# Nicolo2277/Vivim

Measured on AMD Instinct MI355X. Metric: frames/sec fwd+bwd, 256x256 clip=5 3-class, higher is better.
Workload: dtype bf16

## Files before the change

### include/vivim_hip.h

```cpp
#ifndef VIVIM_HIP_H
#define VIVIM_HIP_H

#include <stddef.h>
#include <stdint.h>

#ifdef __cplusplus
extern "C" {
#endif

#define VIVIM_ABI_VERSION 8

typedef enum { VIVIM_F32 = 0, VIVIM_F16 = 1, VIVIM_BF16 = 2 } vivim_dtype_t;

enum {
    VIVIM_OK = 0,
    VIVIM_ERR_INVALID = 1,
    VIVIM_ERR_UNSUPPORTED = 2,
    VIVIM_ERR_LAUNCH = 3
};

typedef struct {
    int32_t batch, dim, seqlen, dstate, n_groups;
    int32_t itype;
    int32_t is_variable_B;
// ... 139 lines not shown
    const void *z;
    const void *dt_bias;
    void *out;
} vivim_state_update_params;

typedef struct {
    int32_t batch, seqlen, channels;
    int32_t itype, otype;
    float eps;
    int64_t x_batch_stride, x_c_stride;
    int64_t y_batch_stride, y_token_stride;
    int64_t dx_batch_stride, dx_c_stride;
    const void *x;
    const void *weight, *bias;
    void *y;
    void *mean, *rstd;
    const void *dy;
    void *dx;
    void *dweight, *dbias;
    void *workspace;
} vivim_layernorm_params;

typedef struct {
    int32_t groups, m, n, k;
    int32_t itype;
    int32_t _pad0;
    int64_t a_group_stride, a_row_stride;
    int64_t b_group_stride, b_row_stride;
    int64_t out_group_stride, out_row_stride;
    const void *a, *b;
    void *out;
} vivim_wgrad_nt_params;

int vivim_abi_version(void);
const char *vivim_last_error(void);

size_t vivim_sizeof(int which);

int vivim_scan_ckpt_len(const vivim_ssm_fwd_params *f);
int vivim_scan_chunk_len(int itype);

size_t vivim_scan_bwd_workspace_bytes(const vivim_ssm_fwd_params *f);
size_t vivim_scan_fwd_workspace_bytes(const vivim_ssm_fwd_params *f);

int vivim_set_tuning(int which, int value);

int vivim_selective_scan_fwd(const vivim_ssm_fwd_params *p, void *stream);
int vivim_selective_scan_bwd(const vivim_ssm_bwd_params *p, void *stream);
int vivim_causal_conv1d_fwd(const vivim_conv_fwd_params *p, void *stream);
int vivim_causal_conv1d_bwd(const vivim_conv_bwd_params *p, void *stream);
int vivim_dwconv_fwd(const vivim_dwconv_params *p, void *stream);
int vivim_dwconv_wgrad(const vivim_dwconv_wgrad_params *p, void *stream);
int vivim_dir_scatter(const vivim_dir_params *p, void *stream);
int vivim_dir_gather(const vivim_dir_params *p, void *stream);
int vivim_causal_conv1d_update(const vivim_conv_update_params *p, void *stream);
int vivim_selective_state_update(const vivim_state_update_params *p, void *stream);
int vivim_layernorm_cm_fwd(const vivim_layernorm_params *p, void *stream);
int vivim_layernorm_cm_bwd(const vivim_layernorm_params *p, void *stream);
size_t vivim_layernorm_bwd_workspace_bytes(const vivim_layernorm_params *p);
int vivim_wgrad_nt(const vivim_wgrad_nt_params *p, void *stream);

size_t vivim_scan_bwd_det_workspace_bytes(const vivim_ssm_fwd_params *f);
size_t vivim_scan_bwd_det_call_workspace_bytes(const vivim_ssm_bwd_params *p);
int vivim_selective_scan_bwd_det(const vivim_ssm_bwd_params *p, void *det_ws, size_t det_ws_bytes, void *stream);

size_t vivim_causal_conv1d_bwd_det_workspace_bytes(const vivim_conv_fwd_params *f);
int vivim_causal_conv1d_bwd_det(const vivim_conv_bwd_params *p, void *det_ws, size_t det_ws_bytes, void *stream);
size_t vivim_dwconv_wgrad_det_workspace_bytes(const vivim_dwconv_wgrad_params *p);
int vivim_dwconv_wgrad_det(const vivim_dwconv_wgrad_params *p, void *det_ws, size_t det_ws_bytes, void *stream);

#ifdef __cplusplus
}
#endif
#endif
```

### vivim_amd/_lib.py

```python
import ctypes
import os
import subprocess

_HERE = os.path.dirname(os.path.abspath(__file__))
CSRC = os.path.join(_HERE, "csrc")
SO_PATH = os.environ.get("VIVIM_LIB") or os.path.join(CSRC, "libvivim_hip.so")

i32, i64, vp = ctypes.c_int32, ctypes.c_int64, ctypes.c_void_p

F32, F16, BF16 = 0, 1, 2


class SsmFwdParams(ctypes.Structure):
    _fields_ = (
        [(n, i32) for n in ("batch", "dim", "seqlen", "dstate", "n_groups", "itype", "is_variable_B",
                            "is_variable_C", "delta_softplus", "_pad0")]
        + [(n, i64) for n in ("u_batch_stride", "u_d_stride", "delta_batch_stride", "delta_d_stride",
                              "z_batch_stride", "z_d_stride", "out_batch_stride", "out_d_stride",
                              "out_z_batch_stride", "out_z_d_stride", "A_d_stride", "A_dstate_stride",
                              "B_batch_stride", "B_group_stride", "B_dstate_stride",
                              "C_batch_stride", "C_group_stride", "C_dstate_stride")]
        + [(n, vp) for n in ("u", "delta", "A", "B", "C", "D", "delta_bias", "z", "out", "out_z", "x", "workspace")]
        + [("workspace_bytes", i64)]
    )
# ... 58 lines not shown


class ConvUpdateParams(ctypes.Structure):
    _fields_ = ([(n, i32) for n in ("batch", "dim", "width", "itype", "wtype", "silu_activation")]
                + [(n, i64) for n in ("x_batch_stride", "x_c_stride", "state_batch_stride", "state_c_stride",
                                      "state_w_stride", "weight_c_stride", "weight_width_stride",
                                      "out_batch_stride", "out_c_stride")]
                + [(n, vp) for n in ("x", "conv_state", "weight", "bias", "out")])


class StateUpdateParams(ctypes.Structure):
    _fields_ = ([(n, i32) for n in ("batch", "dim", "dstate", "itype", "stype", "dt_softplus")]
                + [(n, i64) for n in ("state_batch_stride", "state_d_stride", "state_n_stride", "x_batch_stride",
                                      "x_d_stride", "dt_batch_stride", "dt_d_stride", "A_d_stride", "A_n_stride",
                                      "B_batch_stride", "B_n_stride", "C_batch_stride", "C_n_stride",
                                      "z_batch_stride", "z_d_stride", "out_batch_stride", "out_d_stride")]
                + [(n, vp) for n in ("state", "x", "dt", "A", "B", "C", "D", "z", "dt_bias", "out")])


class LayerNormParams(ctypes.Structure):
    _fields_ = ([(n, i32) for n in ("batch", "seqlen", "channels", "itype", "otype")] + [("eps", ctypes.c_float)]
                + [(n, i64) for n in ("x_batch_stride", "x_c_stride", "y_batch_stride", "y_token_stride",
                                      "dx_batch_stride", "dx_c_stride")]
                + [(n, vp) for n in ("x", "weight", "bias", "y", "mean", "rstd", "dy", "dx", "dweight", "dbias", "workspace")])


class WgradNtParams(ctypes.Structure):
    _fields_ = ([(n, i32) for n in ("groups", "m", "n", "k", "itype", "_pad0")]
                + [(n, i64) for n in ("a_group_stride", "a_row_stride", "b_group_stride", "b_row_stride",
                                      "out_group_stride", "out_row_stride")]
                + [(n, vp) for n in ("a", "b", "out")])


EXPORTS = ("vivim_abi_version", "vivim_last_error", "vivim_scan_chunk_len", "vivim_scan_ckpt_len", "vivim_sizeof",
           "vivim_scan_bwd_workspace_bytes", "vivim_scan_fwd_workspace_bytes", "vivim_set_tuning",
           "vivim_selective_scan_fwd", "vivim_selective_scan_bwd",
           "vivim_causal_conv1d_fwd", "vivim_causal_conv1d_bwd", "vivim_dwconv_fwd", "vivim_dwconv_wgrad",
           "vivim_dir_scatter", "vivim_dir_gather", "vivim_causal_conv1d_update", "vivim_selective_state_update",
           "vivim_layernorm_cm_fwd", "vivim_layernorm_cm_bwd", "vivim_layernorm_bwd_workspace_bytes", "vivim_wgrad_nt",
           "vivim_scan_bwd_det_workspace_bytes", "vivim_scan_bwd_det_call_workspace_bytes", "vivim_selective_scan_bwd_det",
           "vivim_causal_conv1d_bwd_det_workspace_bytes", "vivim_causal_conv1d_bwd_det",
           "vivim_dwconv_wgrad_det_workspace_bytes", "vivim_dwconv_wgrad_det")

_lib = None


def build(force=False):
    if force:
        subprocess.check_call(["make", "-C", CSRC, "clean"])
    subprocess.check_call(["make", "-C", CSRC, "-j4"])
    return SO_PATH


def lib():
    global _lib
    if _lib is None:
        if not os.path.exists(SO_PATH):
            raise ImportError(
                f"{SO_PATH} is missing: run `python -c 'import __graft_entry__ as g; g.build()'` "
                "(or `make -C vivim_amd/csrc`). vivim_amd has no fallback path.")
        import torch
        L = ctypes.CDLL(SO_PATH)
        L.vivim_last_error.restype = ctypes.c_char_p
        L.vivim_sizeof.restype = ctypes.c_size_t
        L.vivim_sizeof.argtypes = [ctypes.c_int]
        L.vivim_set_tuning.restype = ctypes.c_int
        L.vivim_set_tuning.argtypes = [ctypes.c_int, ctypes.c_int]
        L.vivim_scan_ckpt_len.restype = ctypes.c_int
        L.vivim_scan_ckpt_len.argtypes = [ctypes.POINTER(SsmFwdParams)]
        for fn in (L.vivim_scan_bwd_workspace_bytes, L.vivim_scan_fwd_workspace_bytes):
            fn.restype = ctypes.c_size_t
            fn.argtypes = [ctypes.POINTER(SsmFwdParams)]
        for name, st in (("vivim_selective_scan_fwd", SsmFwdParams), ("vivim_selective_scan_bwd", SsmBwdParams),
                         ("vivim_causal_conv1d_fwd", ConvFwdParams), ("vivim_causal_conv1d_bwd", ConvBwdParams),
                         ("vivim_dwconv_fwd", DwConvParams), ("vivim_dwconv_wgrad", DwConvWgradParams),
                         ("vivim_dir_scatter", DirParams), ("vivim_dir_gather", DirParams),
                         ("vivim_causal_conv1d_update", ConvUpdateParams),
                         ("vivim_selective_state_update", StateUpdateParams),
                         ("vivim_layernorm_cm_fwd", LayerNormParams), ("vivim_layernorm_cm_bwd", LayerNormParams),
                         ("vivim_wgrad_nt", WgradNtParams)):
            fn = getattr(L, name)
            fn.argtypes = [ctypes.POINTER(st), vp]
            fn.restype = ctypes.c_int
        L.vivim_scan_bwd_det_workspace_bytes.restype = ctypes.c_size_t
        L.vivim_scan_bwd_det_workspace_bytes.argtypes = [ctypes.POINTER(SsmFwdParams)]
        for name, st in (("vivim_scan_bwd_det_call_workspace_bytes", SsmBwdParams),
                         ("vivim_causal_conv1d_bwd_det_workspace_bytes", ConvFwdParams),
                         ("vivim_dwconv_wgrad_det_workspace_bytes", DwConvWgradParams)):
            getattr(L, name).restype = ctypes.c_size_t
            getattr(L, name).argtypes = [ctypes.POINTER(st)]
        for name, st in (("vivim_selective_scan_bwd_det", SsmBwdParams), ("vivim_causal_conv1d_bwd_det", ConvBwdParams),
                         ("vivim_dwconv_wgrad_det", DwConvWgradParams)):
            getattr(L, name).argtypes = [ctypes.POINTER(st), vp, ctypes.c_size_t, vp]
            getattr(L, name).restype = ctypes.c_int
        L.vivim_layernorm_bwd_workspace_bytes.argtypes = [ctypes.POINTER(LayerNormParams)]
        L.vivim_layernorm_bwd_workspace_bytes.restype = ctypes.c_size_t
        if L.vivim_abi_version() != 8:
            raise ImportError("libvivim_hip.so ABI version mismatch")
        for which, st in enumerate((SsmFwdParams, SsmBwdParams, ConvFwdParams, ConvBwdParams, DwConvParams,
                                    DwConvWgradParams, DirParams, ConvUpdateParams, StateUpdateParams, LayerNormParams,
                                    WgradNtParams)):
            if L.vivim_sizeof(which) != ctypes.sizeof(st):
                raise ImportError(f"struct layout mismatch for {st.__name__}: "
                                  f"C {L.vivim_sizeof(which)} vs ctypes {ctypes.sizeof(st)}")
        _lib = L
    return _lib


_ISIZE = {F32: 4, F16: 2, BF16: 2}


def algorithmic_bytes(name, P):
    if name.startswith("vivim_selective_scan"):
        f = P.f if name.endswith("bwd") else P
        s = _ISIZE[f.itype]
        act = f.batch * f.dim * f.seqlen * s
        bc = (f.batch * f.n_groups * f.dstate * f.seqlen) if f.is_variable_B else f.dim * f.dstate
        has_z = bool(f.z)
        if name.endswith("fwd"):
            n_act = 3 + (2 if has_z else 0)
            return n_act * act + 2 * bc * (s if f.is_variable_B else 4) + 4 * (f.dim * f.dstate + 2 * f.dim)
        n_act = 5 + (3 if has_z else 0) + (1 if (has_z and f.out_z) else 0)
        return (n_act * act + 2 * bc * (s if f.is_variable_B else 4) + 2 * bc * 4
                + 4 * (2 * f.dim * f.dstate + 4 * f.dim))
    if name.endswith("_update"):
        return 0
    if name.startswith("vivim_dir"):
        return 4 * P.batch * P.channels * P.seqlen * _ISIZE[P.itype]
    if name.startswith("vivim_dwconv"):
        act = P.batch * P.depth * P.height * P.width * P.channels * _ISIZE[P.itype]
        return 2 * act + 4 * P.channels * (P.kd * 9 + 1)
    f = P.f if name.endswith("bwd") else P
    s = _ISIZE[f.itype]
    act = f.batch * f.dim * f.seqlen * s
    if name.endswith("fwd"):
        return 2 * act + 4 * f.dim * (f.width + 1)
    return 3 * act + 8 * f.dim * (f.width + 1)


_profile = None
_event_pool = []
_PROFILED = ("vivim_selective_scan_fwd", "vivim_selective_scan_bwd", "vivim_causal_conv1d_fwd",
             "vivim_causal_conv1d_bwd")


def profile_begin(all_kernels=False):
    global _profile
    _profile = ([], bool(all_kernels))


def profile_end():
    global _profile
    rec = _profile[0] if _profile else []
    _profile = None
    out = []
    for name, nbytes, e0, e1 in rec:
        e1.synchronize()
        out.append((name, nbytes, e0.elapsed_time(e1) * 1e-3))
        _event_pool.extend((e0, e1))
    return out

# ... 88 lines not shown
```

### vivim_amd/csrc/capi.hip

```cpp
#include <hip/hip_runtime.h>
#include <stdarg.h>
#include <stdio.h>
#include "../../include/vivim_hip.h"
#include "det.cuh"

namespace vivim {
bool conv_fwd_dispatch(const vivim_conv_fwd_params&, hipStream_t);
bool conv_bwd_dispatch(const vivim_conv_bwd_params&, hipStream_t);
bool conv_cl_fwd_dispatch(const vivim_conv_fwd_params&, hipStream_t);
bool conv_cl_bwd_dispatch(const vivim_conv_bwd_params&, hipStream_t);
bool ssm_fwd_dispatch(const vivim_ssm_fwd_params&, hipStream_t);
bool dwconv_fwd_dispatch(const vivim_dwconv_params&, hipStream_t);
bool dwconv_wgrad_dispatch(const vivim_dwconv_wgrad_params&, hipStream_t);
template <bool GATHER> bool dir_dispatch(const vivim_dir_params&, hipStream_t);
void conv_update_launch(const vivim_conv_update_params&, hipStream_t);
void state_update_launch(const vivim_state_update_params&, hipStream_t);
bool ssm_bwd_dispatch(const vivim_ssm_bwd_params&, hipStream_t);
int scan_chunk_len(int itype);
int scan_ckpt_len(const vivim_ssm_fwd_params&);
size_t scan_bwd_workspace_bytes(const vivim_ssm_fwd_params&);
size_t scan_bwd_det_workspace_bytes(const vivim_ssm_fwd_params&);
size_t scan_bwd_det_call_workspace_bytes(const vivim_ssm_bwd_params&);
size_t conv_bwd_det_slots(const vivim_conv_fwd_params&);
bool conv_bwd_det_launch(const vivim_conv_bwd_params&, hipStream_t);
size_t conv_cl_bwd_det_slots(const vivim_conv_fwd_params&);
bool conv_cl_bwd_det_launch(const vivim_conv_bwd_params&, hipStream_t);
size_t dwconv_wgrad_det_workspace_bytes(const vivim_dwconv_wgrad_params&);
int dwconv_wgrad_det_dispatch(const vivim_dwconv_wgrad_params&, void*, size_t, hipStream_t);
int ssm_bwd_det_dispatch(const vivim_ssm_bwd_params&, void* det_ws, size_t det_ws_bytes, hipStream_t);
bool layernorm_dispatch(const vivim_layernorm_params&, bool bwd, hipStream_t);
size_t layernorm_bwd_workspace_bytes(const vivim_layernorm_params&);
bool wgrad_nt_dispatch(const vivim_wgrad_nt_params&, hipStream_t);
size_t scan_fwd_workspace_bytes(const vivim_ssm_fwd_params&);
}

static thread_local char g_err[512] = "";

static int fail(int code, const char* fmt, ...) {
    va_list ap;
    va_start(ap, fmt);
    vsnprintf(g_err, sizeof(g_err), fmt, ap);
    va_end(ap);
    return code;
}

#define VCHECK(cond)                                                                   \
    do {                                                                               \
        if (!(cond)) return fail(VIVIM_ERR_INVALID, "%s: check failed: %s", __func__, #cond); \
    } while (0)

static int after_launch(const char* what) {
    const hipError_t e = hipGetLastError();
    if (e != hipSuccess) return fail(VIVIM_ERR_LAUNCH, "%s: launch failed: %s", what, hipGetErrorString(e));
    return VIVIM_OK;
}

static bool dtype_ok(int t) { return t == VIVIM_F32 || t == VIVIM_F16 || t == VIVIM_BF16; }

static int check_ssm_fwd(const vivim_ssm_fwd_params* p, bool is_bwd) {
    VCHECK(p != nullptr);
    VCHECK(dtype_ok(p->itype));
    VCHECK(p->batch > 0 && p->dim > 0 && p->seqlen > 0 && p->dstate > 0 && p->n_groups > 0);
    VCHECK(p->dstate <= 256);
    VCHECK(p->dim % p->n_groups == 0);
    VCHECK(p->u && p->delta && p->A && p->B && p->C);
// ... 27 lines not shown
}

extern "C" {

int vivim_set_tuning(int which, int value) {
    if (which < 0 || which > 1 || value < 0) return -1;
    const int prev = which == 0 ? vivim::tuning_fwd_variant() : vivim::tuning_bwd_variant();
    __atomic_store_n(&vivim::g_tune[which], value, __ATOMIC_RELAXED);
    return prev;
}
int vivim_abi_version(void) { return VIVIM_ABI_VERSION; }
const char* vivim_last_error(void) { return g_err; }
int vivim_scan_chunk_len(int itype) { return vivim::scan_chunk_len(itype); }
int vivim_scan_ckpt_len(const vivim_ssm_fwd_params* f) { return f ? vivim::scan_ckpt_len(*f) : 0; }
size_t vivim_scan_bwd_workspace_bytes(const vivim_ssm_fwd_params* f) {
    return f ? vivim::scan_bwd_workspace_bytes(*f) : 0;
}
size_t vivim_scan_fwd_workspace_bytes(const vivim_ssm_fwd_params* f) {
    return f ? vivim::scan_fwd_workspace_bytes(*f) : 0;
}
size_t vivim_sizeof(int which) {
    switch (which) {
        case 0: return sizeof(vivim_ssm_fwd_params);
        case 1: return sizeof(vivim_ssm_bwd_params);
        case 2: return sizeof(vivim_conv_fwd_params);
        case 3: return sizeof(vivim_conv_bwd_params);
        case 4: return sizeof(vivim_dwconv_params);
        case 5: return sizeof(vivim_dwconv_wgrad_params);
        case 6: return sizeof(vivim_dir_params);
        case 7: return sizeof(vivim_conv_update_params);
        case 8: return sizeof(vivim_state_update_params);
        case 9: return sizeof(vivim_layernorm_params);
        case 10: return sizeof(vivim_wgrad_nt_params);
    }
    return 0;
}

int vivim_selective_scan_fwd(const vivim_ssm_fwd_params* p, void* stream) {
    if (int rc = check_ssm_fwd(p, false)) return rc;
    if (!vivim::ssm_fwd_dispatch(*p, static_cast<hipStream_t>(stream)))
        return fail(VIVIM_ERR_UNSUPPORTED, "selective_scan_fwd not implemented for input type %d", p->itype);
    return after_launch("selective_scan_fwd");
}

static int check_ssm_bwd(const vivim_ssm_bwd_params* p) {
    VCHECK(p != nullptr);
    if (int rc = check_ssm_fwd(&p->f, true)) return rc;
    VCHECK(p->dout && p->du && p->ddelta && p->dA && p->dB && p->dC);
    VCHECK((p->f.D == nullptr) == (p->dD == nullptr));
    VCHECK((p->f.delta_bias == nullptr) == (p->ddelta_bias == nullptr));
    VCHECK((p->f.z == nullptr) == (p->dz == nullptr));
    return VIVIM_OK;
}

int vivim_selective_scan_bwd(const vivim_ssm_bwd_params* p, void* stream) {
    if (int rc = check_ssm_bwd(p)) return rc;
    if (!vivim::ssm_bwd_dispatch(*p, static_cast<hipStream_t>(stream)))
        return fail(VIVIM_ERR_UNSUPPORTED, "selective_scan_bwd not implemented for input type %d", p->f.itype);
    return after_launch("selective_scan_bwd");
}

size_t vivim_scan_bwd_det_workspace_bytes(const vivim_ssm_fwd_params* f) {
    return f && f->batch > 0 && f->dim > 0 && f->seqlen > 0 && f->dstate > 0 && f->n_groups > 0
               ? vivim::scan_bwd_det_workspace_bytes(*f) : 0;
}

// ... 226 lines not shown
}

size_t vivim_layernorm_bwd_workspace_bytes(const vivim_layernorm_params* p) {
    return p && p->batch > 0 && p->seqlen > 0 && p->channels > 0 ? vivim::layernorm_bwd_workspace_bytes(*p) : 0;
}

int vivim_layernorm_cm_bwd(const vivim_layernorm_params* p, void* stream) {
    if (int rc = check_layernorm(p)) return rc;
    VCHECK(p->dy && p->dx && (reinterpret_cast<uintptr_t>(p->dx) & 15) == 0);
    const int64_t e = p->itype == VIVIM_F32 ? 4 : 8;
    VCHECK(p->dx_batch_stride % e == 0 && p->dx_c_stride % e == 0);
    if ((p->dweight || p->dbias) && !p->workspace)
        return fail(VIVIM_ERR_INVALID, "layernorm_cm_bwd: dweight / dbias need the workspace (vivim_layernorm_bwd_workspace_bytes)");
    if (!vivim::layernorm_dispatch(*p, true, static_cast<hipStream_t>(stream)))
        return fail(VIVIM_ERR_UNSUPPORTED, "layernorm_cm_bwd not implemented for input type %d / output type %d", p->itype, p->otype);
    return after_launch("layernorm_cm_bwd");
}

int vivim_wgrad_nt(const vivim_wgrad_nt_params* p, void* stream) {
    VCHECK(p != nullptr);
    VCHECK(p->groups > 0 && p->groups <= 65535 && p->m > 0 && p->n > 0 && p->k > 0);
    VCHECK(p->a && p->b && p->out);
    if (p->itype != VIVIM_F16 && p->itype != VIVIM_BF16)
        return fail(VIVIM_ERR_UNSUPPORTED, "wgrad_nt takes f16 or bf16 operands (type %d given): f32 products stay on the library GEMM", p->itype);
    VCHECK(p->k % 8 == 0 && p->a_row_stride % 8 == 0 && p->b_row_stride % 8 == 0 && p->a_group_stride % 8 == 0 &&
           p->b_group_stride % 8 == 0);
    VCHECK((reinterpret_cast<uintptr_t>(p->a) & 15) == 0 && (reinterpret_cast<uintptr_t>(p->b) & 15) == 0);
    VCHECK((int64_t)((p->m + 63) / 64) * ((p->n + 15) / 16) <= 65535);
    if (!vivim::wgrad_nt_dispatch(*p, static_cast<hipStream_t>(stream)))
        return fail(VIVIM_ERR_UNSUPPORTED, "wgrad_nt not implemented for type %d", p->itype);
    return after_launch("wgrad_nt");
}

}
```

### vivim_amd/mamba_simple.py

```python
import math

import torch
import torch.nn as nn
import torch.nn.functional as F

import os

from .dirmap import combine_directions, stack_directions
from .causal_conv1d_interface import causal_conv1d_update
from .selective_scan_interface import mamba_inner_fn_no_out_proj, mamba_inner_grouped_fn_no_out_proj
from .selective_state_update import selective_state_update

_DIRECTIONS = ("", "_b", "_s")
_FUSED = ("conv1d{}.weight", "conv1d{}.bias", "x_proj{}.weight", "dt_proj{}.weight", "dt_proj{}.bias", "A{}_log", "D{}")


class _FusedViews(torch.autograd.Function):

    @staticmethod
    def forward(ctx, nb, *args):
        ctx.nb = nb
        return tuple(b.view_as(b) for b in args[:nb])

    @staticmethod
    def backward(ctx, *gs):
        out = [None] * (1 + ctx.nb)
        for g in gs:
            out += [None, None, None] if g is None else [g[0], g[1], g[2]]
        return tuple(out)


class Mamba(nn.Module):
    def __init__(self, d_model, d_state=16, d_conv=4, expand=2, dt_rank="auto", dt_min=0.001, dt_max=0.1,
                 dt_init="random", dt_scale=1.0, dt_init_floor=1e-4, conv_bias=True, bias=False,
                 use_fast_path=True, layer_idx=None, device=None, dtype=None, bimamba_type="none",
                 nframes=5):
        kw = {"device": device, "dtype": dtype}
        super().__init__()
        assert bimamba_type == "v3", "this fork only builds the tri-directional v3 block (mamba_simple.py:125)"
        self.d_model, self.d_state, self.d_conv, self.expand = d_model, d_state, d_conv, expand
# ... 84 lines not shown
        bufs = self._fused
        views = iter(_FusedViews.apply(len(self._fused_live), *self._fused_args))
        return [None if b is None else next(views) for b in bufs]

    def _inner(self, xz, sfx):
        conv, x_proj, dt_proj = (getattr(self, n + sfx) for n in ("conv1d", "x_proj", "dt_proj"))
        A = -torch.exp(getattr(self, f"A{sfx}_log").float())
        return mamba_inner_fn_no_out_proj(
            xz, conv.weight, conv.bias, x_proj.weight, dt_proj.weight, A, None, None,
            getattr(self, "D" + sfx).float(), delta_bias=dt_proj.bias.float(), delta_softplus=True)

    def forward(self, hidden_states, inference_params=None, nframes=None):
        if inference_params is not None:
            raise NotImplementedError("decode-time inference cache is outside Vivim's path")
        batch, seqlen, _ = hidden_states.shape
        nf = self.nframes if nframes is None else nframes
        if seqlen % nf != 0:
            raise ValueError(f"seqlen {seqlen} is not a multiple of nframes {nf}")
        xz = (self.in_proj.weight @ hidden_states.reshape(batch * seqlen, -1).t()
              ).view(2 * self.d_inner, batch, seqlen).transpose(0, 1)
        if self.in_proj.bias is not None:
            xz = xz + self.in_proj.bias.to(xz.dtype)[:, None]
        hw = seqlen // nf
        if os.environ.get("VIVIM_SEPARATE_DIRECTIONS", "0") == "1" or seqlen % 8 != 0:
            return self._forward_separate(xz, batch, seqlen, nf, hw)
        D = self.d_inner
        xz3 = stack_directions(xz, nf)
        conv_w, conv_b, x_proj_w, dt_proj_w, dt_bias, A_log, Dp = self._fused_params()
        A = -torch.exp(A_log.float()).view(3 * D, self.d_state)
        o3 = mamba_inner_grouped_fn_no_out_proj(
            xz3, conv_w.view(3 * D, self.d_conv), conv_b.view(3 * D) if conv_b is not None else None, x_proj_w, dt_proj_w,
            A, Dp.float().view(3 * D), dt_bias.float().view(3 * D), True).view(batch, 3, D, seqlen)
        y = combine_directions(o3, nf).transpose(1, 2)
        return F.linear(y, self.out_proj.weight, self.out_proj.bias)

    def _forward_separate(self, xz, batch, seqlen, nf, hw):
        out = self._inner(xz, "")
        out_b = self._inner(xz.flip([-1]), "_b").flip([-1])
        xz_s = xz.reshape(batch, 2 * self.d_inner, nf, hw).transpose(2, 3).reshape(batch, 2 * self.d_inner, seqlen)
        out_s = self._inner(xz_s, "_s")
        out_s = out_s.reshape(batch, self.d_inner, hw, nf).transpose(2, 3).reshape(batch, self.d_inner, seqlen)
        y = (out + out_b + out_s).transpose(1, 2) / 3
        return F.linear(y, self.out_proj.weight, self.out_proj.bias)

    def step(self, hidden_states, conv_state, ssm_state):
        assert hidden_states.shape[1] == 1, "Only support decoding with 1 token at a time for now"
        xz = self.in_proj(hidden_states.squeeze(1))
        x, z = xz.chunk(2, dim=-1)
        x = causal_conv1d_update(x.contiguous(), conv_state, self.conv1d.weight.squeeze(1), self.conv1d.bias, self.activation)
        x_db = self.x_proj(x)
        dt, B, C = torch.split(x_db, [self.dt_rank, self.d_state, self.d_state], dim=-1)
        dt = F.linear(dt, self.dt_proj.weight)
        A = -torch.exp(self.A_log.float())
        y = selective_state_update(ssm_state, x, dt, A, B, C, self.D, z=z, dt_bias=self.dt_proj.bias, dt_softplus=True)
        return self.out_proj(y).unsqueeze(1), conv_state, ssm_state

    def allocate_inference_cache(self, batch_size, max_seqlen, dtype=None, **kwargs):
        device = self.out_proj.weight.device
        conv_state = torch.zeros(batch_size, self.d_inner, self.d_conv, device=device,
                                 dtype=self.conv1d.weight.dtype if dtype is None else dtype)
        ssm_state = torch.zeros(batch_size, self.d_inner, self.d_state, device=device,
                                dtype=self.dt_proj.weight.dtype if dtype is None else dtype)
        return conv_state, ssm_state
```

### vivim_amd/vivim.py

```python
import math

import os

import torch
import torch.nn as nn
import torch.nn.functional as F

from . import dwconv as _dw
from . import layernorm as _ln
from .mamba_simple import Mamba


class DropPath(nn.Module):

    def __init__(self, drop_prob=0.0):
        super().__init__()
        self.drop_prob = drop_prob

    def forward(self, x):
        if self.drop_prob == 0.0 or not self.training:
            return x
        keep = 1.0 - self.drop_prob
        mask = x.new_empty((x.shape[0],) + (1,) * (x.dim() - 1)).bernoulli_(keep).div_(keep)
        return x * mask


def _init_weights(m):
    if isinstance(m, nn.Linear):
        nn.init.trunc_normal_(m.weight, std=0.02)
        if m.bias is not None:
            nn.init.constant_(m.bias, 0)
    elif isinstance(m, nn.LayerNorm):
        nn.init.constant_(m.bias, 0)
        nn.init.constant_(m.weight, 1.0)
    elif isinstance(m, nn.Conv2d):
        fan_out = m.kernel_size[0] * m.kernel_size[1] * m.out_channels // m.groups
        m.weight.data.normal_(0, math.sqrt(2.0 / fan_out))
        if m.bias is not None:
            m.bias.data.zero_()


class LayerNorm(nn.Module):
# ... 14 lines not shown
        mean = x.mean(1, keepdim=True)
        var = (x - mean).pow(2).mean(1, keepdim=True)
        x = (x - mean) / torch.sqrt(var + self.eps)
        return self.weight[:, None, None] * x + self.bias[:, None, None]


class DWConv(nn.Module):

    def __init__(self, dim=768):
        super().__init__()
        self.dwconv = nn.Conv3d(dim, dim, 3, 1, 1, bias=True, groups=dim)

    def forward(self, x, nf, H, W):
        B, _, C = x.shape
        if _dw.supported(x, self.dwconv.weight):
            return _dw.depthwise_conv_tokens(x, self.dwconv.weight, self.dwconv.bias, nf, H, W)
        x = self.dwconv(x.transpose(1, 2).view(B, C, nf, H, W))
        return x.flatten(2).transpose(1, 2)


class Mlp(nn.Module):
    def __init__(self, in_features, hidden_features=None, out_features=None, act_layer=nn.GELU, drop=0.0):
        super().__init__()
        out_features = out_features or in_features
        hidden_features = hidden_features or in_features
        self.fc1 = nn.Linear(in_features, hidden_features)
        self.dwconv = DWConv(hidden_features)
        self.act = act_layer()
        self.fc2 = nn.Linear(hidden_features, out_features)
        self.drop = nn.Dropout(drop)
        self.apply(_init_weights)

    def forward(self, x, nf, H, W):
        x = self.fc1(x)
        conv = self.dwconv.dwconv
        if isinstance(self.act, nn.GELU) and self.act.approximate == "none" and _dw.supported(x, conv.weight) \
                and not os.environ.get("VIVIM_NO_DWCONV_GELU"):
            x = self.drop(_dw.depthwise_conv_gelu_tokens(x, conv.weight, conv.bias, nf, H, W))
        else:
            x = self.drop(self.act(self.dwconv(x, nf, H, W)))
        return self.drop(self.fc2(x))


class MambaLayer(nn.Module):

    def __init__(self, dim, d_state=16, d_conv=4, expand=2, mlp_ratio=4, drop=0.0, drop_path=0.0,
                 act_layer=nn.GELU):
        super().__init__()
        self.dim = dim
        self.norm1 = nn.LayerNorm(dim)
        self.mamba = Mamba(d_model=dim, d_state=d_state, d_conv=d_conv, expand=expand, bimamba_type="v3")
        self.drop_path = DropPath(drop_path) if drop_path > 0.0 else nn.Identity()
        self.norm2 = nn.LayerNorm(dim)
        self.mlp = Mlp(in_features=dim, hidden_features=int(dim * mlp_ratio), act_layer=act_layer, drop=drop)
        self.apply(_init_weights)

    @staticmethod
    def _norm(norm, x_flat):
        if (_ln.supported(x_flat, norm.weight) and _ln.worthwhile(x_flat)
                and not os.environ.get("VIVIM_NO_FUSED_LAYERNORM")):
            return _ln.layer_norm_cm(x_flat, norm.weight, norm.bias, norm.eps)
        return norm(x_flat)

    def forward(self, x):
        B, C, nf, H, W = x.shape
        assert C == self.dim
        x_flat = x.reshape(B, C, nf * H * W).transpose(-1, -2)
        x_flat = x_flat + self.drop_path(self.mamba(self._norm(self.norm1, x_flat), nframes=nf))
        x_flat = x_flat + self.drop_path(self.mlp(self._norm(self.norm2, x_flat), nf, H, W))
        return x_flat.transpose(-1, -2).reshape(B, C, nf, H, W)


def _encoder_parts(backbone):
    seg = backbone.segformer
# ... 35 lines not shown
    for m in module.modules():
        dp = getattr(m, "drop_path", None)
        if isinstance(dp, nn.Module) and type(dp).__name__ == "SegformerDropPath":
            m.drop_path = DropPath(float(dp.drop_prob))
            n += 1
    return n


class _Encoder(nn.Module):

    def __init__(self, backbone):
        super().__init__()
        pe, blocks, norms = _encoder_parts(backbone)
        self.patch_embeddings = nn.ModuleList(pe)
        self.block = nn.ModuleList(blocks)
        self.layer_norm = nn.ModuleList(norms)


def _run_block(blk, hs, height, width):
    out = blk(hs, height, width)
    return out[0] if isinstance(out, (tuple, list)) else out


class mamba_block(nn.Module):

    def __init__(self, backbone, in_chans=1, depths=[2, 2, 2, 2], dims=[64, 128, 320, 512],
                 drop_path_rate=0.0, layer_scale_init_value=1e-6, out_indices=[0, 1, 2, 3], mamba_kwargs=None,
                 fast_backbone_dwconv=False):
        super().__init__()
        self.downsample_layers = _Encoder(backbone)
        if fast_backbone_dwconv:
            _swap_backbone_dwconv(self.downsample_layers)
            _swap_backbone_droppath(self.downsample_layers)
        dp_rates = [x.item() for x in torch.linspace(0, drop_path_rate, sum(depths))]
        mk = mamba_kwargs or {}
        self.stages = nn.ModuleList()
        for i in range(len(dims)):
            self.stages.append(nn.Sequential(*[nn.Sequential(MambaLayer(dim=dims[i], drop_path=dp_rates[i], **mk))
                                               for _ in range(depths[i])]))
        self.out_indices = out_indices

    def forward_features(self, x):
        bz, nf = x.shape[:2]
        hs = x.reshape(bz * nf, *x.shape[-3:])
        outs = []
        enc = self.downsample_layers
        for embed, blocks, _norm, mam_stage in zip(enc.patch_embeddings, enc.block, enc.layer_norm, self.stages):
            hs, height, width = embed(hs)
            for blk in blocks:
                hs = _run_block(blk, hs, height, width)
            hs = hs.reshape(bz * nf, height, width, -1).permute(0, 3, 1, 2).contiguous()
            hs = hs.reshape(bz, nf, *hs.shape[-3:]).transpose(1, 2)
            hs = mam_stage(hs)
            hs = hs.transpose(1, 2).reshape(bz * nf, hs.shape[1], height, width)
            outs.append(hs)
        return tuple(outs)

    def forward(self, x):
        return self.forward_features(x)


def segformer_b3_config(num_labels=150):
    from transformers import SegformerConfig
    return SegformerConfig(num_channels=3, num_encoder_blocks=4, depths=[3, 4, 18, 3], sr_ratios=[8, 4, 2, 1],
                           hidden_sizes=[64, 128, 320, 512], patch_sizes=[7, 3, 3, 3], strides=[4, 2, 2, 2],
                           num_attention_heads=[1, 2, 5, 8], mlp_ratios=[4, 4, 4, 4], decoder_hidden_size=768,
                           num_labels=num_labels)


def segformer_b3_random(num_labels=150):
    from transformers import SegformerForSemanticSegmentation
    return SegformerForSemanticSegmentation(segformer_b3_config(num_labels))


class Vivim(nn.Module):

    def __init__(self, in_chans=3, out_chans=3, depths=[2, 2, 2, 2], feat_size=[64, 128, 320, 512],
                 drop_path_rate=0.2, layer_scale_init_value=1e-6, hidden_size: int = 768, norm_name="instance",
                 conv_block: bool = True, res_block: bool = True, spatial_dims=2, with_edge=False,
                 dropout_rate=0.3, backbone=None, mamba_kwargs=None, fast_backbone_dwconv=False) -> None:
        super().__init__()
        self.hidden_size = hidden_size
        self.in_chans, self.out_chans = in_chans, out_chans
        self.depths, self.feat_size = depths, feat_size
        self.drop_path_rate = drop_path_rate
        self.layer_scale_init_value = layer_scale_init_value
        self.dropout_rate = dropout_rate
        self.spatial_dims = spatial_dims
        if backbone is None:
            from transformers import SegformerForSemanticSegmentation
            backbone = SegformerForSemanticSegmentation.from_pretrained("nvidia/segformer-b3-finetuned-ade-512-512")
        self.encoder = mamba_block(backbone, in_chans, depths=depths, dims=feat_size,
                                   drop_path_rate=drop_path_rate, mamba_kwargs=mamba_kwargs,
                                   fast_backbone_dwconv=fast_backbone_dwconv)
        self.decoder = backbone.decode_head
        self.feature_dropout = nn.Dropout2d(dropout_rate)
        self.out = nn.Conv2d(768, out_chans, kernel_size=1)
        self.with_edge = with_edge
        if with_edge:
            self.edgeocr_cls_head = nn.Conv2d(64, 1, kernel_size=1, stride=1, padding=0, bias=True)

    def _decoder_projections(self):
        dec = self.decoder
        return dec.linear_c if hasattr(dec, "linear_c") else dec.linear_projections

    def decode(self, encoder_hidden_states, bz, nf):
        batch_size = encoder_hidden_states[-1].shape[0]
        size0 = encoder_hidden_states[0].shape[2:]
        feats = ()
        for state, mlp in zip(encoder_hidden_states, self._decoder_projections()):
            height, width = state.shape[2], state.shape[3]
            state = mlp(state).permute(0, 2, 1).reshape(batch_size, -1, height, width)
            state = F.interpolate(state, size=size0, mode="bilinear", align_corners=False)
            if torch.rand(1).item() > 0.5:
                state = F.dropout(state, p=self.dropout_rate / 2, training=self.training)
            feats += (state,)
        hidden = self.decoder.linear_fuse(torch.cat(feats[::-1], dim=1))
        hidden = self.decoder.activation(self.decoder.batch_norm(hidden))
        hidden = self.decoder.dropout(self.decoder.dropout(hidden))
        hidden = self.feature_dropout(hidden)
        return self.out(hidden)

    def forward(self, x_in):
        bz, nf, nc, h, w = x_in.shape
        outs = self.encoder(x_in)
        logits = F.interpolate(self.decode(outs, bz, nf), size=(h, w), mode="bilinear", align_corners=False)
        if self.with_edge:
            edge = F.interpolate(self.edgeocr_cls_head(outs[0]), size=(h, w), mode="bilinear", align_corners=False)
# ... 3 lines not shown
```

### vivim_amd/wgrad.py

```python
import torch

from . import _lib

_ITYPE = {torch.float16: _lib.F16, torch.bfloat16: _lib.BF16}
MIN_TOKENS = 8192


def supported(a, b):
    if _lib.deterministic():
        return False
    if not (a.is_cuda and a.dim() == 3 and b.dim() == 3 and a.dtype in _ITYPE and b.dtype == a.dtype
            and a.shape[0] == b.shape[0] and a.shape[2] == b.shape[2]):
        return False
    ok = lambda t: (t.stride(2) == 1 and t.stride(1) % 8 == 0 and t.stride(0) % 8 == 0 and t.data_ptr() % 16 == 0)
    return a.shape[2] % 8 == 0 and a.shape[2] >= MIN_TOKENS and ok(a) and ok(b) and a.shape[0] <= 65535


def wgrad_nt(a, b):
    G, M, K = a.shape
    N = b.shape[1]
    out = _lib.zeros(G * M * N, a.device).view(G, M, N)
    P = _lib.WgradNtParams()
    P.groups, P.m, P.n, P.k, P.itype = G, M, N, K, _ITYPE[a.dtype]
    P.a_group_stride, P.a_row_stride = a.stride(0), a.stride(1)
    P.b_group_stride, P.b_row_stride = b.stride(0), b.stride(1)
    P.out_group_stride, P.out_row_stride = M * N, N
    P.a, P.b, P.out = a.data_ptr(), b.data_ptr(), out.data_ptr()
    if a.device.index == torch.cuda.current_device():
        _lib.call("vivim_wgrad_nt", P, torch.cuda.current_stream().cuda_stream)
    else:
        with torch.cuda.device(a.device):
            _lib.call("vivim_wgrad_nt", P, torch.cuda.current_stream().cuda_stream)
    return out
```

Baseline: 223.5.

## Add fused MFMA weight-gradient kernel with bias reduction for linear layers

Adds a custom HIP split-K GEMM kernel that computes the linear-layer weight gradient dy^T·x with bf16/f16 MFMA, using LDS transpose reads and a register prefetch pipeline. The bias gradient is reduced in the same pass over dy, and partial sums are combined with fp32 atomics. A custom autograd linear routes fc1/fc2, out_proj, backbone and decoder linears through this path when there are enough tokens. This replaces a library GEMM plus a separate column sum, which may help the small-M/N, large-K shapes. The cost is atomic accumulation, a zero-init buffer and non-deterministic summation order.

```diff
diff --git a/include/vivim_hip.h b/include/vivim_hip.h
--- a/include/vivim_hip.h
+++ b/include/vivim_hip.h
@@ -195,6 +195,16 @@
     void *out;
 } vivim_wgrad_nt_params;
 
+typedef struct {
+    int32_t m, n, k;
+    int32_t itype;
+    int64_t dy_row_stride, x_row_stride;
+    int64_t out_row_stride;
+    const void *dy, *x;
+    void *out;
+    void *dbias;
+} vivim_wgrad_tn_params;
+
 int vivim_abi_version(void);
 const char *vivim_last_error(void);
 
@@ -222,6 +232,7 @@
 int vivim_layernorm_cm_bwd(const vivim_layernorm_params *p, void *stream);
 size_t vivim_layernorm_bwd_workspace_bytes(const vivim_layernorm_params *p);
 int vivim_wgrad_nt(const vivim_wgrad_nt_params *p, void *stream);
+int vivim_wgrad_tn(const vivim_wgrad_tn_params *p, void *stream);
 
 size_t vivim_scan_bwd_det_workspace_bytes(const vivim_ssm_fwd_params *f);
 size_t vivim_scan_bwd_det_call_workspace_bytes(const vivim_ssm_bwd_params *p);
diff --git a/vivim_amd/_lib.py b/vivim_amd/_lib.py
--- a/vivim_amd/_lib.py
+++ b/vivim_amd/_lib.py
@@ -114,12 +114,19 @@
                 + [(n, vp) for n in ("a", "b", "out")])
 
 
+class WgradTnParams(ctypes.Structure):
+    _fields_ = ([(n, i32) for n in ("m", "n", "k", "itype")]
+                + [(n, i64) for n in ("dy_row_stride", "x_row_stride", "out_row_stride")]
+                + [(n, vp) for n in ("dy", "x", "out", "dbias")])
+
+
 EXPORTS = ("vivim_abi_version", "vivim_last_error", "vivim_scan_chunk_len", "vivim_scan_ckpt_len", "vivim_sizeof",
            "vivim_scan_bwd_workspace_bytes", "vivim_scan_fwd_workspace_bytes", "vivim_set_tuning",
            "vivim_selective_scan_fwd", "vivim_selective_scan_bwd",
            "vivim_causal_conv1d_fwd", "vivim_causal_conv1d_bwd", "vivim_dwconv_fwd", "vivim_dwconv_wgrad",
            "vivim_dir_scatter", "vivim_dir_gather", "vivim_causal_conv1d_update", "vivim_selective_state_update",
            "vivim_layernorm_cm_fwd", "vivim_layernorm_cm_bwd", "vivim_layernorm_bwd_workspace_bytes", "vivim_wgrad_nt",
+           "vivim_wgrad_tn",
            "vivim_scan_bwd_det_workspace_bytes", "vivim_scan_bwd_det_call_workspace_bytes", "vivim_selective_scan_bwd_det",
            "vivim_causal_conv1d_bwd_det_workspace_bytes", "vivim_causal_conv1d_bwd_det",
            "vivim_dwconv_wgrad_det_workspace_bytes", "vivim_dwconv_wgrad_det")
@@ -160,7 +167,7 @@
                          ("vivim_causal_conv1d_update", ConvUpdateParams),
                          ("vivim_selective_state_update", StateUpdateParams),
                          ("vivim_layernorm_cm_fwd", LayerNormParams), ("vivim_layernorm_cm_bwd", LayerNormParams),
-                         ("vivim_wgrad_nt", WgradNtParams)):
+                         ("vivim_wgrad_nt", WgradNtParams), ("vivim_wgrad_tn", WgradTnParams)):
             fn = getattr(L, name)
             fn.argtypes = [ctypes.POINTER(st), vp]
             fn.restype = ctypes.c_int
@@ -181,7 +188,7 @@
             raise ImportError("libvivim_hip.so ABI version mismatch")
         for which, st in enumerate((SsmFwdParams, SsmBwdParams, ConvFwdParams, ConvBwdParams, DwConvParams,
                                     DwConvWgradParams, DirParams, ConvUpdateParams, StateUpdateParams, LayerNormParams,
-                                    WgradNtParams)):
+                                    WgradNtParams, WgradTnParams)):
             if L.vivim_sizeof(which) != ctypes.sizeof(st):
                 raise ImportError(f"struct layout mismatch for {st.__name__}: "
                                   f"C {L.vivim_sizeof(which)} vs ctypes {ctypes.sizeof(st)}")
@@ -209,6 +216,10 @@
         return 0
     if name.startswith("vivim_dir"):
         return 4 * P.batch * P.channels * P.seqlen * _ISIZE[P.itype]
+    if name.startswith("vivim_wgrad"):
+        if name.endswith("_tn"):
+            return P.k * (P.m + P.n) * _ISIZE[P.itype] + 4 * P.m * (P.n + 1)
+        return P.groups * (P.k * (P.m + P.n) * _ISIZE[P.itype] + 4 * P.m * P.n)
     if name.startswith("vivim_dwconv"):
         act = P.batch * P.depth * P.height * P.width * P.channels * _ISIZE[P.itype]
         return 2 * act + 4 * P.channels * (P.kd * 9 + 1)
diff --git a/vivim_amd/csrc/capi.hip b/vivim_amd/csrc/capi.hip
--- a/vivim_amd/csrc/capi.hip
+++ b/vivim_amd/csrc/capi.hip
@@ -31,6 +31,8 @@
 bool layernorm_dispatch(const vivim_layernorm_params&, bool bwd, hipStream_t);
 size_t layernorm_bwd_workspace_bytes(const vivim_layernorm_params&);
 bool wgrad_nt_dispatch(const vivim_wgrad_nt_params&, hipStream_t);
+bool wgrad_tn_dispatch(const vivim_wgrad_tn_params&, hipStream_t);
+int64_t wgrad_tn_tiles(const vivim_wgrad_tn_params&);
 size_t scan_fwd_workspace_bytes(const vivim_ssm_fwd_params&);
 }
 
@@ -124,6 +126,7 @@
         case 8: return sizeof(vivim_state_update_params);
         case 9: return sizeof(vivim_layernorm_params);
         case 10: return sizeof(vivim_wgrad_nt_params);
+        case 11: return sizeof(vivim_wgrad_tn_params);
     }
     return 0;
 }
@@ -416,4 +419,21 @@
     return after_launch("wgrad_nt");
 }
 
-}
+int vivim_wgrad_tn(const vivim_wgrad_tn_params* p, void* stream) {
+    VCHECK(p != nullptr);
+    VCHECK(p->m > 0 && p->n > 0 && p->k > 0);
+    VCHECK(p->dy && p->x && p->out);
+    if (p->itype != VIVIM_F16 && p->itype != VIVIM_BF16)
+        return fail(VIVIM_ERR_UNSUPPORTED, "wgrad_tn takes f16 or bf16 operands (type %d given): f32 products stay on the library GEMM", p->itype);
+    VCHECK(p->m % 8 == 0 && p->n % 8 == 0);
+    VCHECK(p->dy_row_stride % 8 == 0 && p->x_row_stride % 8 == 0 && p->dy_row_stride >= p->m && p->x_row_stride >= p->n);
+    VCHECK(p->out_row_stride >= p->n);
+    VCHECK((reinterpret_cast<uintptr_t>(p->dy) & 15) == 0 && (reinterpret_cast<uintptr_t>(p->x) & 15) == 0);
+    VCHECK((reinterpret_cast<uintptr_t>(p->out) & 3) == 0 && (reinterpret_cast<uintptr_t>(p->dbias) & 3) == 0);
+    VCHECK(vivim::wgrad_tn_tiles(*p) <= 65535);
+    if (!vivim::wgrad_tn_dispatch(*p, static_cast<hipStream_t>(stream)))
+        return fail(VIVIM_ERR_UNSUPPORTED, "wgrad_tn not implemented for type %d", p->itype);
+    return after_launch("wgrad_tn");
+}
+
+}
diff --git a/vivim_amd/csrc/wgrad_tn.hip b/vivim_amd/csrc/wgrad_tn.hip
--- /dev/null
+++ b/vivim_amd/csrc/wgrad_tn.hip
@@ -0,0 +1,199 @@
+#include "common.cuh"
+
+namespace vivim {
+
+typedef __attribute__((ext_vector_type(8))) __bf16 tn_bf8;
+typedef __attribute__((ext_vector_type(8))) _Float16 tn_h8;
+typedef __attribute__((ext_vector_type(4))) float tn_f4;
+typedef __attribute__((ext_vector_type(4))) short tn_s4;
+
+template <typename T> struct TnFrag;
+template <> struct TnFrag<bf16_t> {
+    typedef tn_bf8 type;
+    static __device__ __forceinline__ tn_f4 mma(type a, type b, tn_f4 c) { return __builtin_amdgcn_mfma_f32_16x16x32_bf16(a, b, c, 0, 0, 0); }
+    static __device__ __forceinline__ float f32(uint32_t bits16) { return __uint_as_float(bits16 << 16); }
+};
+template <> struct TnFrag<f16_t> {
+    typedef tn_h8 type;
+    static __device__ __forceinline__ tn_f4 mma(type a, type b, tn_f4 c) { return __builtin_amdgcn_mfma_f32_16x16x32_f16(a, b, c, 0, 0, 0); }
+    static __device__ __forceinline__ float f32(uint32_t bits16) {
+        union { uint16_t u; _Float16 h; } v;
+        v.u = (uint16_t)bits16;
+        return (float)v.h;
+    }
+};
+
+constexpr int kTnThreads = 256;
+constexpr int kTnDepth = 3;
+constexpr int kTnPad = 16;
+
+typedef __attribute__((address_space(3))) tn_s4 tn_lds_s4;
+
+template <typename T>
+__device__ __forceinline__ typename TnFrag<T>::type tn_read_frag(const T* img, int pitch, int c0, int lane) {
+    const int g = lane >> 4, q = (lane & 15) >> 2, pp = lane & 3;
+    const T* p0 = img + (4 * g + q) * pitch + c0 + 4 * pp;
+    union { tn_s4 h[2]; typename TnFrag<T>::type f; } u;
+    u.h[0] = __builtin_amdgcn_ds_read_tr16_b64_v4i16((tn_lds_s4*)(p0));
+    u.h[1] = __builtin_amdgcn_ds_read_tr16_b64_v4i16((tn_lds_s4*)(p0 + 16 * pitch));
+    return u.f;
+}
+
+template <typename T, int MF, int NF>
+__global__ void __launch_bounds__(kTnThreads) wgrad_tn_kernel(const vivim_wgrad_tn_params p, const int steps_per_split, const int col_tiles) {
+    typedef typename TnFrag<T>::type frag;
+    constexpr int TM = 32 * MF, TN = 32 * NF, PA = TM + kTnPad, PB = TN + kTnPad;
+    constexpr int LA = TM / 64, LB = TN / 64;
+    constexpr int CRA = TM / 8, CRB = TN / 8;
+    constexpr int IMG = 32 * (PA + PB);
+    static_assert(MF % 2 == 0 && NF % 2 == 0, "a step's piece must be a whole number of loads per thread");
+    static_assert(2 * IMG * sizeof(T) >= kTnThreads * 8 * sizeof(float), "the bias reduction reuses the images");
+    __shared__ __attribute__((aligned(16))) T lds[2 * IMG];
+
+    const int tid = threadIdx.x, lane = tid & 63, wave = tid >> 6;
+    const int wm = wave >> 1, wn = wave & 1;
+    const int rt = blockIdx.y / col_tiles, ct = blockIdx.y - rt * col_tiles;
+    const int m0 = rt * TM, n0 = ct * TN;
+    const bool do_bias = p.dbias != nullptr && ct == 0;
+
+    const int nsteps = (p.k + 31) / 32;
+    const int s0 = blockIdx.x * steps_per_split, s1 = min(nsteps, s0 + steps_per_split);
+
+    const T* __restrict__ dy = static_cast<const T*>(p.dy);
+    const T* __restrict__ x = static_cast<const T*>(p.x);
+    const int cha = 8 * (tid % CRA), chb = 8 * (tid % CRB);
+    const bool a_in = m0 + cha < p.m, b_in = n0 + chb < p.n;
+    const u32x4 zero = {0u, 0u, 0u, 0u};
+    auto load_a = [&](int s, int j) -> u32x4 {
+        const int tok = 32 * s + (tid + kTnThreads * j) / CRA;
+        const bool ok = a_in && s < s1 && tok < p.k;
+        const u32x4 v = *reinterpret_cast<const u32x4*>(ok ? dy + (int64_t)tok * p.dy_row_stride + m0 + cha : dy);
+        return ok ? v : zero;
+    };
+    auto load_b = [&](int s, int j) -> u32x4 {
+        const int tok = 32 * s + (tid + kTnThreads * j) / CRB;
+        const bool ok = b_in && s < s1 && tok < p.k;
+        const u32x4 v = *reinterpret_cast<const u32x4*>(ok ? x + (int64_t)tok * p.x_row_stride + n0 + chb : x);
+        return ok ? v : zero;
+    };
+
+    tn_f4 acc[MF][NF];
+#pragma unroll
+    for (int i = 0; i < MF; ++i)
+#pragma unroll
+        for (int j = 0; j < NF; ++j) acc[i][j] = tn_f4{0.f, 0.f, 0.f, 0.f};
+    float bsum[8];
+#pragma unroll
+    for (int e = 0; e < 8; ++e) bsum[e] = 0.f;
+
+    u32x4 ra[kTnDepth][LA], rb[kTnDepth][LB];
+#pragma unroll
+    for (int d = 0; d < kTnDepth - 1; ++d) {
+#pragma unroll
+        for (int j = 0; j < LA; ++j) ra[d][j] = load_a(s0 + d, j);
+#pragma unroll
+        for (int j = 0; j < LB; ++j) rb[d][j] = load_b(s0 + d, j);
+    }
+    int buf = 0;
+    for (int s = s0; s < s1; s += kTnDepth) {
+#pragma unroll
+        for (int h = 0; h < kTnDepth; ++h) {
+            constexpr int D1 = kTnDepth - 1;
+            const int nxt = (h + D1) % kTnDepth;
+#pragma unroll
+            for (int j = 0; j < LA; ++j) ra[nxt][j] = load_a(s + h + D1, j);
+#pragma unroll
+            for (int j = 0; j < LB; ++j) rb[nxt][j] = load_b(s + h + D1, j);
+            T* imga = lds + buf * IMG;
+            T* imgb = imga + 32 * PA;
+#pragma unroll
+            for (int j = 0; j < LA; ++j)
+                *reinterpret_cast<u32x4*>(imga + ((tid + kTnThreads * j) / CRA) * PA + cha) = ra[h][j];
+#pragma unroll
+            for (int j = 0; j < LB; ++j)
+                *reinterpret_cast<u32x4*>(imgb + ((tid + kTnThreads * j) / CRB) * PB + chb) = rb[h][j];
+            if (do_bias) {
+#pragma unroll
+                for (int j = 0; j < LA; ++j)
+#pragma unroll
+                    for (int e = 0; e < 4; ++e) {
+                        bsum[2 * e] += TnFrag<T>::f32(ra[h][j][e] & 0xffffu);
+                        bsum[2 * e + 1] += TnFrag<T>::f32(ra[h][j][e] >> 16);
+                    }
+            }
+            lds_barrier();
+            frag fa[MF], fb[NF];
+#pragma unroll
+            for (int i = 0; i < MF; ++i) fa[i] = tn_read_frag<T>(imga, PA, 16 * (wm * MF + i), lane);
+#pragma unroll
+            for (int j = 0; j < NF; ++j) fb[j] = tn_read_frag<T>(imgb, PB, 16 * (wn * NF + j), lane);
+#pragma unroll
+            for (int i = 0; i < MF; ++i)
+#pragma unroll
+                for (int j = 0; j < NF; ++j) acc[i][j] = TnFrag<T>::mma(fa[i], fb[j], acc[i][j]);
+            buf ^= 1;
+        }
+    }
+    float* __restrict__ out = static_cast<float*>(p.out);
+    const int r = lane & 15, kq = lane >> 4;
+#pragma unroll
+    for (int i = 0; i < MF; ++i)
+#pragma unroll
+        for (int j = 0; j < NF; ++j) {
+            const int col = n0 + 16 * (wn * NF + j) + r;
+#pragma unroll
+            for (int e = 0; e < 4; ++e) {
+                const int row = m0 + 16 * (wm * MF + i) + 4 * kq + e;
+                if (row < p.m && col < p.n) atomicAdd(out + (int64_t)row * p.out_row_stride + col, acc[i][j][e]);
+            }
+        }
+    if (do_bias) {
+        float* red = reinterpret_cast<float*>(lds);
+        __syncthreads();
+#pragma unroll
+        for (int e = 0; e < 8; ++e) red[e * kTnThreads + tid] = bsum[e];
+        __syncthreads();
+        if (tid < TM && m0 + tid < p.m) {
+            float sum = 0.f;
+            for (int k = tid >> 3; k < kTnThreads; k += CRA) sum += red[(tid & 7) * kTnThreads + k];
+            atomicAdd(static_cast<float*>(p.dbias) + m0 + tid, sum);
+        }
+    }
+}
+
+template <typename T, int MF, int NF>
+static void wgrad_tn_launch_tile(const vivim_wgrad_tn_params& p, hipStream_t stream) {
+    constexpr int TM = 32 * MF, TN = 32 * NF;
+    const int row_tiles = (p.m + TM - 1) / TM, col_tiles = (p.n + TN - 1) / TN;
+    const int nsteps = (p.k + 31) / 32;
+    const int64_t tiles = (int64_t)row_tiles * col_tiles;
+    int splits = (int)std::min<int64_t>(std::max<int64_t>(1, 1024 / tiles), std::max(1, nsteps / 8));
+    const int sps = (nsteps + splits - 1) / splits;
+    splits = (nsteps + sps - 1) / sps;
+    const dim3 grid(splits, row_tiles * col_tiles), block(kTnThreads);
+    hipLaunchKernelGGL((wgrad_tn_kernel<T, MF, NF>), grid, block, 0, stream, p, sps, col_tiles);
+}
+
+template <typename T>
+static void wgrad_tn_launch(const vivim_wgrad_tn_params& p, hipStream_t stream) {
+    const bool bm = p.m > 64, bn = p.n > 64;
+    if (bm && bn) wgrad_tn_launch_tile<T, 4, 4>(p, stream);
+    else if (bm) wgrad_tn_launch_tile<T, 4, 2>(p, stream);
+    else if (bn) wgrad_tn_launch_tile<T, 2, 4>(p, stream);
+    else wgrad_tn_launch_tile<T, 2, 2>(p, stream);
+}
+
+int64_t wgrad_tn_tiles(const vivim_wgrad_tn_params& p) {
+    const int tm = p.m > 64 ? 128 : 64, tn = p.n > 64 ? 128 : 64;
+    return (int64_t)((p.m + tm - 1) / tm) * ((p.n + tn - 1) / tn);
+}
+
+bool wgrad_tn_dispatch(const vivim_wgrad_tn_params& p, hipStream_t stream) {
+    switch (p.itype) {
+        case VIVIM_BF16: wgrad_tn_launch<bf16_t>(p, stream); return true;
+        case VIVIM_F16: wgrad_tn_launch<f16_t>(p, stream); return true;
+    }
+    return false;
+}
+
+}
diff --git a/vivim_amd/linear.py b/vivim_amd/linear.py
--- /dev/null
+++ b/vivim_amd/linear.py
@@ -0,0 +1,78 @@
+import os
+
+import torch
+import torch.nn as nn
+import torch.nn.functional as F
+
+from . import _lib
+from . import wgrad as _wg
+
+_HALF = (torch.bfloat16, torch.float16)
+
+
+class _LinearFn(torch.autograd.Function):
+    @staticmethod
+    def forward(ctx, x, weight, bias, dtype):
+        x2 = x.reshape(-1, x.shape[-1])
+        fused = bias is not None and (x.dim() == 2 or x.is_contiguous())
+        x2, w = x2.to(dtype), weight.to(dtype)
+        b = None if bias is None else bias.to(dtype)
+        if fused or b is None:
+            y2 = F.linear(x2, w, b)
+        else:
+            y2 = torch.mm(x2, w.t()).add_(b)
+        ctx.save_for_backward(x2, w)
+        ctx.x_shape = x.shape
+        ctx.has_bias = bias is not None
+        ctx.param_dtype = weight.dtype
+        ctx.bias_dtype = None if bias is None else bias.dtype
+        return y2.view(*x.shape[:-1], weight.shape[0])
+
+    @staticmethod
+    def backward(ctx, dy):
+        x2, w = ctx.saved_tensors
+        dy2 = dy.reshape(-1, dy.shape[-1])
+        if dy2.dtype != w.dtype:
+            dy2 = dy2.to(w.dtype)
+        dx = torch.mm(dy2, w).view(ctx.x_shape) if ctx.needs_input_grad[0] else None
+        dw = db = None
+        want_b = ctx.has_bias and ctx.needs_input_grad[2]
+        if ctx.needs_input_grad[1] and _wg.supported_tn(x2, dy2):
+            dw, db = _wg.wgrad_tn(dy2, x2, want_b)
+            if dw.dtype != ctx.param_dtype:
+                dw = dw.to(ctx.param_dtype)
+            if want_b and db.dtype != ctx.bias_dtype:
+                db = db.to(ctx.bias_dtype)
+        else:
+            if ctx.needs_input_grad[1]:
+                dw = torch.mm(dy2.t(), x2).to(ctx.param_dtype)
+            if want_b:
+                db = dy2.sum(0).to(ctx.bias_dtype)
+        return dx, dw, db, None
+
+
+def linear(x, weight, bias=None):
+    if x.numel() < _wg.MIN_TOKENS_TN * x.shape[-1] or not x.is_cuda or os.environ.get("VIVIM_NO_LINEAR_WGRAD"):
+        return F.linear(x, weight, bias)
+    dtype = torch.get_autocast_dtype("cuda") if torch.is_autocast_enabled("cuda") else x.dtype
+    if (dtype not in _HALF or not (torch.is_grad_enabled() and weight.requires_grad) or weight.device != x.device
+            or weight.shape[0] % 8 or weight.shape[1] % 8 or x.dim() < 2 or x.numel() == 0
+            or (dtype != weight.dtype and not torch.is_autocast_enabled("cuda"))
+            or (bias is not None and bias.device != x.device) or _lib.deterministic()):
+        return F.linear(x, weight, bias)
+    return _LinearFn.apply(x, weight, bias, dtype)
+
+
+class WgradLinear(nn.Linear):
+
+    def forward(self, input):
+        return linear(input, self.weight, self.bias)
+
+
+def swap_linears(module):
+    n = 0
+    for m in module.modules():
+        if type(m) is nn.Linear:
+            m.__class__ = WgradLinear
+            n += 1
+    return n
diff --git a/vivim_amd/mamba_simple.py b/vivim_amd/mamba_simple.py
--- a/vivim_amd/mamba_simple.py
+++ b/vivim_amd/mamba_simple.py
@@ -6,6 +6,7 @@
 
 import os
 
+from . import linear as _lin
 from .dirmap import combine_directions, stack_directions
 from .causal_conv1d_interface import causal_conv1d_update
 from .selective_scan_interface import mamba_inner_fn_no_out_proj, mamba_inner_grouped_fn_no_out_proj
@@ -156,7 +157,7 @@
             xz3, conv_w.view(3 * D, self.d_conv), conv_b.view(3 * D) if conv_b is not None else None, x_proj_w, dt_proj_w,
             A, Dp.float().view(3 * D), dt_bias.float().view(3 * D), True).view(batch, 3, D, seqlen)
         y = combine_directions(o3, nf).transpose(1, 2)
-        return F.linear(y, self.out_proj.weight, self.out_proj.bias)
+        return _lin.linear(y, self.out_proj.weight, self.out_proj.bias)
 
     def _forward_separate(self, xz, batch, seqlen, nf, hw):
         out = self._inner(xz, "")
@@ -165,7 +166,7 @@
         out_s = self._inner(xz_s, "_s")
         out_s = out_s.reshape(batch, self.d_inner, hw, nf).transpose(2, 3).reshape(batch, self.d_inner, seqlen)
         y = (out + out_b + out_s).transpose(1, 2) / 3
-        return F.linear(y, self.out_proj.weight, self.out_proj.bias)
+        return _lin.linear(y, self.out_proj.weight, self.out_proj.bias)
 
     def step(self, hidden_states, conv_state, ssm_state):
         assert hidden_states.shape[1] == 1, "Only support decoding with 1 token at a time for now"
diff --git a/vivim_amd/vivim.py b/vivim_amd/vivim.py
--- a/vivim_amd/vivim.py
+++ b/vivim_amd/vivim.py
@@ -8,6 +8,7 @@
 
 from . import dwconv as _dw
 from . import layernorm as _ln
+from . import linear as _lin
 from .mamba_simple import Mamba
 
 
@@ -88,14 +89,14 @@
         self.apply(_init_weights)
 
     def forward(self, x, nf, H, W):
-        x = self.fc1(x)
+        x = _lin.linear(x, self.fc1.weight, self.fc1.bias)
         conv = self.dwconv.dwconv
         if isinstance(self.act, nn.GELU) and self.act.approximate == "none" and _dw.supported(x, conv.weight) \
                 and not os.environ.get("VIVIM_NO_DWCONV_GELU"):
             x = self.drop(_dw.depthwise_conv_gelu_tokens(x, conv.weight, conv.bias, nf, H, W))
         else:
             x = self.drop(self.act(self.dwconv(x, nf, H, W)))
-        return self.drop(self.fc2(x))
+        return self.drop(_lin.linear(x, self.fc2.weight, self.fc2.bias))
 
 
 class MambaLayer(nn.Module):
@@ -197,6 +198,7 @@
         if fast_backbone_dwconv:
             _swap_backbone_dwconv(self.downsample_layers)
             _swap_backbone_droppath(self.downsample_layers)
+            _lin.swap_linears(self.downsample_layers)
         dp_rates = [x.item() for x in torch.linspace(0, drop_path_rate, sum(depths))]
         mk = mamba_kwargs or {}
         self.stages = nn.ModuleList()
@@ -259,6 +261,8 @@
                                    drop_path_rate=drop_path_rate, mamba_kwargs=mamba_kwargs,
                                    fast_backbone_dwconv=fast_backbone_dwconv)
         self.decoder = backbone.decode_head
+        if fast_backbone_dwconv:
+            _lin.swap_linears(self._decoder_projections())
         self.feature_dropout = nn.Dropout2d(dropout_rate)
         self.out = nn.Conv2d(768, out_chans, kernel_size=1)
         self.with_edge = with_edge
diff --git a/vivim_amd/wgrad.py b/vivim_amd/wgrad.py
--- a/vivim_amd/wgrad.py
+++ b/vivim_amd/wgrad.py
@@ -4,12 +4,13 @@
 
 _ITYPE = {torch.float16: _lib.F16, torch.bfloat16: _lib.BF16}
 MIN_TOKENS = 8192
+MIN_TOKENS_TN = 960
 
 
 def supported(a, b):
     if _lib.deterministic():
         return False
-    if not (a.is_cuda and a.dim() == 3 and b.dim() == 3 and a.dtype in _ITYPE and b.dtype == a.dtype
+    if not (a.is_cuda and b.is_cuda and a.device == b.device and a.dim() == 3 and b.dim() == 3 and a.dtype in _ITYPE and b.dtype == a.dtype
             and a.shape[0] == b.shape[0] and a.shape[2] == b.shape[2]):
         return False
     ok = lambda t: (t.stride(2) == 1 and t.stride(1) % 8 == 0 and t.stride(0) % 8 == 0 and t.data_ptr() % 16 == 0)
@@ -32,3 +33,33 @@
         with torch.cuda.device(a.device):
             _lib.call("vivim_wgrad_nt", P, torch.cuda.current_stream().cuda_stream)
     return out
+
+
+def supported_tn(x, dy):
+    if _lib.deterministic():
+        return False
+    if not (x.is_cuda and dy.is_cuda and x.device == dy.device and x.dim() == 2 and dy.dim() == 2 and x.dtype in _ITYPE
+            and dy.dtype == x.dtype and x.shape[0] == dy.shape[0]):
+        return False
+    ok = lambda t: (t.stride(1) == 1 and t.stride(0) % 8 == 0 and t.stride(0) >= t.shape[1] and t.shape[1] % 8 == 0
+                    and t.data_ptr() % 16 == 0)
+    return x.shape[0] >= max(1, MIN_TOKENS_TN) and ok(x) and ok(dy)
+
+
+def wgrad_tn(dy, x, want_bias=True):
+    K, M = dy.shape
+    N = x.shape[1]
+    buf = _lib.zeros(M * N + (M if want_bias else 0), dy.device)
+    out = buf[:M * N].view(M, N)
+    dbias = buf[M * N:] if want_bias else None
+    P = _lib.WgradTnParams()
+    P.m, P.n, P.k, P.itype = M, N, K, _ITYPE[dy.dtype]
+    P.dy_row_stride, P.x_row_stride, P.out_row_stride = dy.stride(0), x.stride(0), N
+    P.dy, P.x, P.out = dy.data_ptr(), x.data_ptr(), out.data_ptr()
+    P.dbias = dbias.data_ptr() if want_bias else None
+    if dy.device.index == torch.cuda.current_device():
+        _lib.call("vivim_wgrad_tn", P, torch.cuda.current_stream().cuda_stream)
+    else:
+        with torch.cuda.device(dy.device):
+            _lib.call("vivim_wgrad_tn", P, torch.cuda.current_stream().cuda_stream)
+    return out, dbias
```

New measurement: 190.8. 14.6% lower.
